# ZYM-PKU/UDiffText

Measured on AMD Instinct MI355X. Metric: 512x512 50-step denoised images/sec (UDiffText hot path: conditioner + 50 CFG Euler steps + VAE decode), higher is better.
Workload: dtype bf16; 1 GPU; 512x512, 50 Euler/DDIM(eta 0) steps, CFG 5.0, 9-char labels, noise_iters 0; global batch 4 per step sharded over 1 GPU(s) = 4 images per GPU in micro-batches of 4: every UNet call runs ONE batch of 4 (8 samples with CFG); 3 such batch(es) in flight per GPU on separate launch streams; BASELINE.json configs[1]; global_batch=4, weights=synthetic (name-keyed recipe), 1361.2 M parameters, launch=hipGraph replay of the sampler steps, in_flight=3, batches_per_unet_call=1

## Files before the change

udifftext_amd/csrc/gemm.hip:

```cpp
#include "common.h"
#include <stdio.h>
#include <stdlib.h>
#include <string.h>
#include <atomic>
#include <cmath>

hipError_t udt_lean_launch_gemm(int cfg, const void* lparams, int smem, int G, int geglu, int ln, hipStream_t s);
hipError_t udt_lean_launch_conv3(const void* c3params, hipStream_t s);

namespace {
#include "tile_common.h"

struct GemmParams {
  const uint16_t* a;
  const uint16_t* a2;
  const uint16_t* w;
  const uint16_t* zero;
  const float* bias;
  const uint16_t* res;
  const float* rowvec;
  void* out;
  const float* colscale;
  const float* in_scsh;
  float* colstats;
// ... 709 lines not shown
  if ((reinterpret_cast<uintptr_t>(d->a) | reinterpret_cast<uintptr_t>(d->w) | reinterpret_cast<uintptr_t>(d->out)) & 15) return false;
  return true;
}

bool lean_plan(const udt_gemm_desc* d, LeanPlan& t, bool want_stats) {
  const int mode = lean_mode();
  if (mode == 0) return false;
  constexpr int unsupported = UDT_GEMM_OUT_F32 | UDT_GEMM_RELU | UDT_GEMM_TRANSPOSED | UDT_GEMM_SILU_OUT;
  if (d->flags & unsupported) return false;
  const bool conv1 = (d->flags & UDT_GEMM_CONV) != 0;
  if (conv1 && (d->ksize != 1 || d->stride != 1 || d->upsample || d->pad_t != 0 || d->pad_l != 0 || d->Hout != d->Hin ||
                d->Wout != d->Win || d->C1 % BK != 0 || d->C2 % BK != 0 || d->ln_colsum || (d->flags & UDT_GEMM_GEGLU)))
    return false;
  const bool mx8 = (d->flags & UDT_GEMM_MX8) != 0;
  const bool emit = d->q8_out != nullptr;
  if (d->batch > 1 || d->in_scsh || (d->colscale != nullptr) != mx8) return false;
  const bool geglu = (d->flags & UDT_GEMM_GEGLU) != 0;
  const bool ln = d->ln_colsum != nullptr;
  if (want_stats && (geglu || ln || !lean_stats_enabled())) return false;
  if (mx8 || emit) {
    if (conv1 || d->rowvec || mode == 0 || (mode > 0 && mode != 1)) return false;
    if (mx8 && (!d->a_scale || d->K % 128 != 0 || d->lda % 16 != 0 || (d->ldw > 0 && d->ldw % 16 != 0))) return false;
    if (mx8 && ln && (!d->rowstat_in || d->rowstat_in_parts <= 0)) return false;
    if (!mx8 && geglu) return false;
    if (mx8 && geglu && !(ln && emit)) return false;
    if (mx8 && !geglu && ln && emit && d->rowstat_out) return false;
    if (emit && (want_stats || !d->q8_scale || d->ld_q8 % 8 != 0 || d->N % (geglu ? 64 : 32) != 0)) return false;
    if (d->rowstat_out && (!emit || geglu)) return false;
    if (d->q8_fixed_col > 0 && (!emit || geglu || d->q8_fixed_col % 32 != 0 || !(d->q8_fixed_mul > 0.f))) return false;
    if ((reinterpret_cast<uintptr_t>(d->q8_out) | reinterpret_cast<uintptr_t>(d->colscale)) & 15) return false;
  } else if (d->rowstat_out || d->rowstat_in) {
    return false;
  }
// ... 36 lines not shown
  if (!geglu && d->N % 160 == 0 && d->N % 128 != 0 && t.cfg == 1) t.cfg = 5;
  if (mode <= 0 && d->N >= 768 && (long long)((d->M + 255) / 256) * ((d->N + 255) / 256) >= 2LL * device_cus() &&
      (d->cu_share <= 1 || lean256_under_lanes())) t.cfg = 6;
  }
  t.stats_rows = 0;
  if (want_stats) {
    if (t.cfg != 1 && t.cfg != 5) {
      if (mode > 0) return false;
      t.cfg = (d->N % 160 == 0 && d->N % 128 != 0) ? 5 : 1;
    }
    if (mx8) t.cfg = 1;
    t.stats_rows = t.cfg == 1 ? 64 : 32;
    const int rpb = d->rows_per_batch > 0 ? d->rows_per_batch : d->M;
    if (rpb % t.stats_rows != 0) return false;
  }
  switch (t.cfg) {
    case 1: t.nw = 4; t.bm = 128; t.bn = 128; t.smem = 2 * (128 + 128) * ROW_BYTES; break;
    case 5: t.nw = 4; t.bm = 128; t.bn = 160; t.smem = 128 * 160 * 4; break;
    case 6: t.nw = 8; t.bm = 256; t.bn = 256; t.smem = 2 * (256 + 256) * ROW_BYTES; break;
    default: return false;
  }
  {
    const int epi = (t.cfg == 6 ? t.bm * t.bn : t.bm * t.bn * 4) + ((ln && t.cfg != 5) ? t.bm * 8 : 0);
    if (t.smem < epi) t.smem = epi;
  }
  t.tiles_m = (d->M + t.bm - 1) / t.bm;
  t.tiles_n = (d->N + t.bn - 1) / t.bn;
  t.tiles = t.tiles_m * t.tiles_n;
  t.nkt = d->K / KT;
  int slots = device_cus() * ((t.cfg == 1 || t.cfg == 5) ? 2 : 1) / share_of(d);
  if (slots < 1) slots = 1;
  int sk = 1;
// ... 210 lines not shown
  LeanPlan lt;
  return lean_plan(d, lt, d->colstats != nullptr) ? 1 : 0;
}

extern "C" int32_t udt_gemm_rowstat_parts(const udt_gemm_desc* d) {
  if (!d || d->M <= 0 || d->N <= 0 || d->K <= 0) return 0;
  udt_gemm_desc t = *d;
  alignas(16) static const uint64_t probe_dst[2] = {0, 0};
  if (!t.q8_out) { t.q8_out = const_cast<uint64_t*>(probe_dst); t.q8_scale = const_cast<uint64_t*>(probe_dst); if (t.ld_q8 <= 0) t.ld_q8 = (t.N + 15) / 16 * 16; }
  LeanPlan lt;
  if (!lean_plan(&t, lt, false) || lt.cfg != 1 || (d->flags & UDT_GEMM_GEGLU)) return 0;
  return (d->N + 63) / 64;
}
extern "C" int32_t udt_gemm_in_scsh_ok(const udt_gemm_desc* d) {
  if (!d || d->K <= 0 || d->K % BK != 0) return 0;
  c3p::Geo ge;
  return conv3p_geometry(d, ge, true) ? 1 : 0;
}

extern "C" int32_t udt_gemm_up4_ok(const udt_gemm_desc* d) {
  if (!d || d->upsample != 2) return 0;
  lg::C3Params c3;
  return lean_conv_plan(d, c3, d->colstats != nullptr) ? 1 : 0;
}

extern "C" int udt_gn_silu_conv3x3_fwd(const udt_gemm_desc* d, void* workspace, size_t workspace_bytes, void* stream) {
  if (!d || !(d->flags & UDT_GEMM_CONV) || d->ksize != 3 || d->stride != 1 || d->pad_t != 1 || d->pad_l != 1 || !d->in_scsh)
    return UDT_ERR_BAD_ARG;
  return udt_gemm(d, workspace, workspace_bytes, stream);
}
// ... 23 lines not shown
    }
  }
  if (use_gemm8(d)) {
    TilePlan t8 = plan_tiles8(d);
    if (!t8.fixup) return 0;
    return G8_HEADER_BYTES + (size_t)t8.G * t8.bm * t8.bn * sizeof(float);
  }
  TilePlan t = plan_tiles(d);
  if (t.bm != 256 || !t.fixup) return 0;
  return G8_HEADER_BYTES + (size_t)t.G * 2 * SLAB_FLOATS * sizeof(float);
}

extern "C" int udt_gemm(const udt_gemm_desc* d, void* workspace, size_t workspace_bytes, void* stream) {
  if (!d || !d->a || !d->w) return UDT_ERR_BAD_ARG;
  if (d->M <= 0 || d->N <= 0 || d->K <= 0) return UDT_ERR_BAD_SHAPE;
  if (d->K % k_tile(d) != 0) return UDT_ERR_BAD_SHAPE;
  if (d->N % 4 != 0) return UDT_ERR_BAD_SHAPE;
  const bool mx8 = (d->flags & UDT_GEMM_MX8) != 0;
  if (mx8 || d->q8_out || d->rowstat_out || d->rowstat_in) {
    LeanPlan lt8;
    if (!lean_plan(d, lt8, d->colstats != nullptr)) return UDT_ERR_BAD_ARG;
  } else if (d->colscale) {
    return UDT_ERR_BAD_ARG;
  }
  const bool conv = (d->flags & UDT_GEMM_CONV) != 0;
  const bool trans = (d->flags & UDT_GEMM_TRANSPOSED) != 0;
  const int batch = d->batch > 0 ? d->batch : 1;
  if (conv) {
    if (d->ksize != 1 && d->ksize != 3) return UDT_ERR_BAD_SHAPE;
    if (d->C1 <= 0 || d->C1 % BK != 0 || d->C2 % BK != 0) return UDT_ERR_BAD_SHAPE;
// ... 97 lines not shown
      lp.kt_split = (conv1 && d->C2 > 0) ? d->C1 / BK : lt.nkt;
      lp.a2_bytes = (unsigned)((long long)d->M * (conv1 ? d->C2 : 0) * 2);
      lp.alpha = d->alpha; lp.ln_eps = d->ln_eps;
      lp.tiles_m = lt.tiles_m; lp.tiles_n = lt.tiles_n; lp.n_block = lt.n_block; lp.tiles = lt.tiles;
      lp.nkt = lt.nkt; lp.splitk = lt.splitk; lp.kt_per = lt.kt_per;
      lp.a_bytes = (unsigned)((long long)d->M * lp.lda * elem_bytes(d));
      lp.w_bytes = (unsigned)((long long)d->N * p.ldw * elem_bytes(d));
      lp.a_scale = mx8 ? reinterpret_cast<const uint32_t*>(d->a_scale) : nullptr;
      lp.colscale = d->colscale;
      lp.rowstat_in = d->rowstat_in; lp.rowstat_in_parts = d->rowstat_in_parts;
      lp.q8_out = reinterpret_cast<uint8_t*>(d->q8_out); lp.q8_scale = reinterpret_cast<uint32_t*>(d->q8_scale); lp.ld_q8 = d->ld_q8;
      lp.rowstat_out = d->rowstat_out;
      lp.q8_fixed_col = d->q8_fixed_col > 0 ? d->q8_fixed_col : 0x7fffffff;
      lp.q8_fixed_mul = d->q8_fixed_mul;
      lp.G = lt.G;
      lp.counters = nullptr; lp.slabs = nullptr;
      if (lt.splitk > 1) {
        if (!workspace || workspace_bytes < lean_workspace(lt)) return UDT_ERR_WORKSPACE;
        lp.counters = reinterpret_cast<int*>(workspace);
        lp.slabs = reinterpret_cast<float*>(reinterpret_cast<char*>(workspace) + G8_HEADER_BYTES);
      }
      UdtProfScope profl(cls, s);
      if (profl.rec) {
        char tag[96];
        snprintf(tag, sizeof(tag), "lean%d%s%s M=%d N=%d K=%d fl=0x%x ln=%d tile=%dx%d units=%d splitk=%d", lt.cfg, mx8 ? "-mx8" : "", d->q8_out ? "+q8" : "",
                 d->M, d->N, d->K, d->flags, d->ln_colsum ? 1 : 0, lt.bm, lt.bn, lt.tiles * lt.splitk, lt.splitk);
        udt_prof_tag(profl.rec, tag);
      }
      const bool geglu = (d->flags & UDT_GEMM_GEGLU) != 0, ln = d->ln_colsum != nullptr;
      hipError_t el;
      el = udt_lean_launch_gemm(lt.cfg, &lp, lt.smem, lt.G, geglu ? 1 : 0, ln ? 1 : 0, s);
      if (el != hipSuccess) return udt_set_hip_error(el);
      return UDT_OK;
    }
  }
  if (d->ln_colsum) return UDT_ERR_BAD_ARG;
  {
    lg::C3Params c3;
    if (lean_conv_plan(d, c3, d->colstats != nullptr)) {
      c3.colstats = d->colstats;
      c3.a = p.a; c3.w = p.w; c3.bias = p.bias; c3.res = p.res; c3.rowvec = p.rowvec; c3.out = reinterpret_cast<uint16_t*>(d->out);
// ... 145 lines not shown
```

udifftext_amd/csrc/lean.h:

```cpp
#pragma once

namespace lg {

using g8::wait_vm;
UDT_DEVINL void raw_barrier() {
  asm volatile("s_waitcnt lgkmcnt(0)" ::: "memory");
  __builtin_amdgcn_s_barrier();
  asm volatile("" ::: "memory");
}
using g8::buf_lds16;
using g8::OOB;

typedef __attribute__((ext_vector_type(2))) __bf16 bf2_t;
UDT_DEVINL float dot2_bf16(uint32_t a, uint32_t b, float c) {
  return __builtin_amdgcn_fdot2_f32_bf16(__builtin_bit_cast(bf2_t, a), __builtin_bit_cast(bf2_t, b), c, false);
}

template <int CPR, int RPI>
UDT_DEVINL void wave_colstats(char* wl, int lane, const float (&cs)[8], const float (&cq)[8], float* dst, bool col_ok) {
#pragma unroll
  for (int h = 0; h < 2; ++h) {
    f32x4 a = {cs[4 * h + 0], cs[4 * h + 1], cs[4 * h + 2], cs[4 * h + 3]};
    f32x4 b = {cq[4 * h + 0], cq[4 * h + 1], cq[4 * h + 2], cq[4 * h + 3]};
    *reinterpret_cast<f32x4*>(wl + lane * 64 + h * 16) = a;
// ... 12 lines not shown
        const f32x4 a = *reinterpret_cast<const f32x4*>(src + h * 16);
        const f32x4 b = *reinterpret_cast<const f32x4*>(src + 32 + h * 16);
#pragma unroll
        for (int e = 0; e < 4; ++e) { ts[4 * h + e] += a[e]; tq[4 * h + e] += b[e]; }
      }
    }
#pragma unroll
    for (int h = 0; h < 4; ++h) {
      f32x4 v = {ts[2 * h], tq[2 * h], ts[2 * h + 1], tq[2 * h + 1]};
      *reinterpret_cast<f32x4*>(dst + h * 4) = v;
    }
  }
}

template <int NW, int WGM, int WGN, int TM, int TN, int NST, bool GEGLU, bool LN, int TMB = TM, bool STATS = false, bool FP8 = false,
          bool EMIT = false>
__global__ void __launch_bounds__(NW * 64, 2) lgemm_kernel(const LParams p) {
  static_assert(!STATS || (!GEGLU && !LN), "statistics-emitting epilogue: plain linears / 1x1 convolutions");
  static_assert(!FP8 || NST == 2, "the fp8 loop is written for the two-stage ring");
  static_assert(!EMIT || (TN * 4) % 4 == 0, "a 32-column block = 4 lanes of the row layout");
  constexpr int EB = FP8 ? 1 : 2;
  static_assert(TM % TMB == 0, "epilogue passes of TMB row tiles");
  static_assert(WGM * WGN == NW, "wave grid");
  static_assert(!GEGLU || TN == 2, "GEGLU pairs the two 32-column tiles of a wave");
  constexpr int BM = WGM * TM * 32, BN = WGN * TN * 32;
  constexpr int A_BYTES = BM * ROW_BYTES, B_BYTES = BN * ROW_BYTES, STAGE_BYTES = A_BYTES + B_BYTES;
  constexpr int A_PIECES = BM / 8, B_PIECES = BN / 8;
  constexpr int A_INSTR = (A_PIECES + NW - 1) / NW, B_INSTR = (B_PIECES + NW - 1) / NW;
  constexpr int LPT = A_INSTR + B_INSTR;
  constexpr int WROWS = TM * 32, WCOLS = TN * 32;
  constexpr int EROW = WCOLS * 4;
  constexpr int EPI_WAVE = TMB * 32 * EROW;
// ... 47 lines not shown
    const int koff = (pslot ^ ((row >> 1) & 7)) * 8;
    const int m = m0 + row;
    a_voff[i] = (m < p.M) ? (unsigned)((long long)m * p.lda * EB + koff * 2) : OOB;
    a2_voff[i] = (m < p.M) ? (unsigned)(((long long)m * p.lda2 + koff) * 2) : OOB;
  }
#pragma unroll
  for (int i = 0; i < B_INSTR; ++i) {
    int idx = wave + NW * i;
    while (idx >= B_PIECES) idx -= NW;
    w_piece[i] = idx;
    const int row = idx * 8 + l3;
    const int koff = (pslot ^ ((row >> 1) & 7)) * 8;
    const int n = n0 + row;
    w_voff[i] = (n < p.N) ? (unsigned)((long long)n * p.ldw * EB + koff * 2) : OOB;
  }
  auto stage = [&](int st, int kt) {
    char* abuf = smem + st * STAGE_BYTES;
    char* bbuf = abuf + A_BYTES;
    if (kt < p.kt_split) {
#pragma unroll
      for (int i = 0; i < A_INSTR; ++i) buf_lds16(rsrc_a, abuf + a_piece[i] * 1024, a_voff[i], kt * ROW_BYTES);
    } else {
#pragma unroll
      for (int i = 0; i < A_INSTR; ++i) buf_lds16(rsrc_a2, abuf + a_piece[i] * 1024, a2_voff[i], (kt - p.kt_split) * ROW_BYTES);
    }
#pragma unroll
    for (int i = 0; i < B_INSTR; ++i) buf_lds16(rsrc_w, bbuf + w_piece[i] * 1024, w_voff[i], kt * ROW_BYTES);
  };

#pragma unroll
  for (int s = 0; s < NST - 1; ++s)
    if (s < nk) stage(s, kreal(s));
  const uint32_t* asp[TM];
  uint32_t asc_nxt[TM];
  if constexpr (FP8) {
#pragma unroll
    for (int tm = 0; tm < TM; ++tm) {
      int m = m0 + row0 + tm * 32 + l31;
      if (m >= p.M) m = p.M - 1;
      asp[tm] = p.a_scale + m;
      asc_nxt[tm] = (nk > 0) ? asp[tm][(long long)kreal(0) * p.M] : 0x7f7f7f7fu;
    }
// ... 71 lines not shown
        for (int tn = 0; tn < TN; ++tn) acc[tm][tn] = mfma32_mx8<2>(wf[1][tn], xf[1][tm], acc[tm][tn], asc[tm]);
      if constexpr (TM * TN <= 5) {
        __builtin_amdgcn_sched_group_barrier(0x100, 4 * (TM + TN), 0);
        __builtin_amdgcn_sched_group_barrier(0x008, 2 * TM * TN, 0);
      }
    } else {
    bf16x8_t xf[4][TM], wf[4][TN];
#pragma unroll
    for (int ks = 0; ks < 4; ++ks) {
      const int slot = ((ks * 2 + hi) ^ swz) << 4;
#pragma unroll
      for (int t = 0; t < TM; ++t) xf[ks][t] = lds_read_frag(abuf + a_frag_row + t * 32 * ROW_BYTES + slot);
#pragma unroll
      for (int t = 0; t < TN; ++t) wf[ks][t] = lds_read_frag(bbuf + b_frag_row + t * 32 * ROW_BYTES + slot);
    }
#pragma unroll
    for (int ks = 0; ks < 4; ++ks) {
#pragma unroll
      for (int tm = 0; tm < TM; ++tm)
#pragma unroll
        for (int tn = 0; tn < TN; ++tn) acc[tm][tn] = mfma32(wf[ks][tn], xf[ks][tm], acc[tm][tn]);
      if constexpr (LN) {
        if (wn == 0) {
#pragma unroll
          for (int tm = 0; tm < TM; ++tm) {
            const u32x4 v = __builtin_bit_cast(u32x4, xf[ks][tm]);
#pragma unroll
            for (int j = 0; j < 4; ++j) {
              rs[tm] = dot2_bf16(v[j], 0x3f803f80u, rs[tm]);
              rq[tm] = dot2_bf16(v[j], v[j], rq[tm]);
            }
          }
        }
      }
    }
    if constexpr (TM * TN <= 5) {
      __builtin_amdgcn_sched_group_barrier(0x100, 4 * (TM + TN), 0);
      __builtin_amdgcn_sched_group_barrier(0x008, 4 * TM * TN, 0);
    }
    }
    st = st + 1;
    if (st >= NST) st = 0;
  }
  raw_barrier();

  if (p.splitk > 1) {
    f32x4* slab = reinterpret_cast<f32x4*>(p.slabs + (long long)unit * (BM * BN));
#pragma unroll
    for (int tm = 0; tm < TM; ++tm)
#pragma unroll
      for (int tn = 0; tn < TN; ++tn)
// ... 668 lines not shown
```

udifftext_amd/csrc/lean.hip:

```cpp
#include "common.h"
#include <stdio.h>
#include <stdlib.h>
#include <atomic>

namespace {
#include "tile_common.h"
#include "lean_params.h"
#include "lean.h"
#include "wide.h"
#include "rowres.h"

template <int NW, int WGM, int WGN, int TM, int TN, int NST, int TMB = TM>
hipError_t launch_lean(const lg::LParams& lp, int smem, int G, bool geglu, bool ln, hipStream_t s) {
  static AttrOnce once[5];
  const void* fn;
  const bool stats = lp.colstats != nullptr;
  if constexpr (NW == 4 && NST == 2) {
    if (stats) {
      fn = (const void*)lg::lgemm_kernel<NW, WGM, WGN, TM, TN, NST, false, false, TMB, true>;
      hipError_t e = once[4].ensure(fn, smem);
      if (e != hipSuccess) return e;
      void* args[] = {const_cast<lg::LParams*>(&lp)};
      return hipLaunchKernel(fn, dim3(G), dim3(NW * 64), args, smem, s);
    }
  }
  if (stats) return hipErrorInvalidValue;
  if constexpr (TN == 2) {
    fn = geglu ? (ln ? (const void*)lg::lgemm_kernel<NW, WGM, WGN, TM, TN, NST, true, true, TMB> : (const void*)lg::lgemm_kernel<NW, WGM, WGN, TM, TN, NST, true, false, TMB>)
               : (ln ? (const void*)lg::lgemm_kernel<NW, WGM, WGN, TM, TN, NST, false, true, TMB> : (const void*)lg::lgemm_kernel<NW, WGM, WGN, TM, TN, NST, false, false, TMB>);
  } else {
    fn = ln ? (const void*)lg::lgemm_kernel<NW, WGM, WGN, TM, TN, NST, false, true, TMB> : (const void*)lg::lgemm_kernel<NW, WGM, WGN, TM, TN, NST, false, false, TMB>;
  }
  hipError_t e = once[(geglu ? 2 : 0) + (ln ? 1 : 0)].ensure(fn, smem);
  if (e != hipSuccess) return e;
  void* args[] = {const_cast<lg::LParams*>(&lp)};
  return hipLaunchKernel(fn, dim3(G), dim3(NW * 64), args, smem, s);
}

template <bool GEGLU, bool LN, bool STATS, bool FP8, bool EMIT>
hipError_t launch_lean_mx8_k(const lg::LParams& lp, int smem, int G, hipStream_t s) {
  static AttrOnce once;
// ... 83 lines not shown
```

udifftext_amd/csrc/lean_params.h:

```cpp
#pragma once

namespace lg {

struct LParams {
  const uint16_t* a;
  const uint16_t* a2;
  const uint16_t* w;
  const float* bias;
  const uint16_t* res;
  const float* rowvec;
  const float* ln_s;
  uint16_t* out;
  int M, N, K;
  int lda, ldw, ldo, ldr, ldrv, rows_per_batch;
  float alpha, ln_eps;
  int tiles_m, tiles_n, n_block, tiles;
  int nkt;
  int splitk, kt_per;
  unsigned a_bytes, w_bytes;
  int kt_split, lda2;
  unsigned a2_bytes;
  int G;
  int* counters;
  float* slabs;
  float* colstats;
  const uint32_t* a_scale;
  const float* colscale;
  const float* rowstat_in;
  int rowstat_in_parts;
  uint8_t* q8_out;
  uint32_t* q8_scale;
  int ld_q8;
  int q8_fixed_col;
  float q8_fixed_mul;
  float* rowstat_out;
};

struct C3Params {
  const uint16_t* a;
  const uint16_t* w;
  const float* bias;
  const uint16_t* res;
  const float* rowvec;
  uint16_t* out;
  int N, C;
  int B, H, W;
  int ldw, ldo, ldr, ldrv;
  float alpha;
  int tiles_x, tiles_y, tiles_m, tiles_n, n_block, tiles;
  int chunks, splitk, ch_per;
// ... 13 lines not shown
```

udifftext_amd/ops.py:

```python
from __future__ import annotations

import contextlib
import ctypes as C
import os
import threading
from typing import NamedTuple, Optional, Sequence

import torch

from . import lib as L

WORKSPACE_BYTES = 96 << 20


class Workspace:

    def __init__(self, device, nbytes: int = WORKSPACE_BYTES):
        if torch.device(device).type != "cuda":
            raise L.UdtError("udifftext_amd workspaces live on the GPU (no CPU fallback)")
        self.buf = torch.zeros(nbytes, dtype=torch.uint8, device=device)

    def check(self, stream: Optional[int] = None) -> None:
        L.check(L.load().udt_check_async_error(self.buf.data_ptr(), self.buf.numel(), _stream() if stream is None else stream),
                "udt_check_async_error")
# ... 59 lines not shown


def _bf16(t: torch.Tensor) -> None:
    if t.dtype != torch.bfloat16:
        raise ValueError(f"expected bf16 tensor, got {t.dtype}")


def gemm_desc(**kw) -> L.GemmDesc:
    d = L.GemmDesc()
    d.batch = 1
    d.alpha = 1.0
    d.cu_share = _ctx.cu_share
    for k, v in kw.items():
        setattr(d, k, v)
    return d


def run_gemm(d: L.GemmDesc, device, fused_gn: bool = False) -> None:
    lib = L.load()
    need = lib.udt_gemm_workspace_bytes(C.byref(d))
    ws_ptr, ws_bytes = None, 0
    if need:
        ws = _ws(need, device)
        ws_ptr, ws_bytes = ws.data_ptr(), ws.numel()
    if fused_gn:
        L.check(lib.udt_gn_silu_conv3x3_fwd(C.byref(d), ws_ptr, ws_bytes, _stream()), "udt_gn_silu_conv3x3_fwd")
    else:
        L.check(lib.udt_gemm(C.byref(d), ws_ptr, ws_bytes, _stream()), "udt_gemm")


# ... 49 lines not shown
    lib = L.load()
    parts = lib.udt_gemm_rowstat_parts(C.byref(d)) if rowstats else 0
    if not lib.udt_gemm_q8_ok(C.byref(d)) or (rowstats and parts <= 0):
        d.q8_out, d.q8_scale, d.ld_q8, d.q8_fixed_col = None, None, 0, 0
        return None
    if rowstats:
        st = torch.empty((parts, M, 2), dtype=torch.float32, device=device)
        d.rowstat_out = st.data_ptr()
        q = Mx8Act(q.data, q.scale, st)
    return q


def linear(x: torch.Tensor, w: torch.Tensor, bias: Optional[torch.Tensor] = None, *, out: Optional[torch.Tensor] = None,
           residual: Optional[torch.Tensor] = None, rowvec: Optional[torch.Tensor] = None, rows_per_batch: int = 0,
           flags: int = 0, alpha: float = 1.0, n_out: Optional[int] = None, colstats: bool = False,
           emit_q8: bool = False, emit_rowstats: bool = False) -> torch.Tensor:
    _bf16(x); _bf16(w)
    K = x.shape[-1]
    x2 = x.reshape(-1, K) if x.is_contiguous() else x
    assert x2.dim() == 2 and x2.stride(1) == 1
    M = x2.shape[0]
    N = w.shape[0] if n_out is None else n_out
    assert w.shape[1] == K and w.is_contiguous()
    n_cols = N // 2 if (flags & L.GEMM_GEGLU) else N
    if out is None:
        dt = torch.float32 if (flags & L.GEMM_OUT_F32) else torch.bfloat16
        if flags & L.GEMM_TRANSPOSED:
            assert rows_per_batch > 0
            out = torch.empty((M // rows_per_batch, N, rows_per_batch), dtype=dt, device=x.device)
        else:
            out = torch.empty((M, n_cols), dtype=dt, device=x.device)
    ldo = out.stride(0) if not (flags & L.GEMM_TRANSPOSED) else 0
    d = gemm_desc(a=_ptr(x2), w=_ptr(w), bias=_ptr(bias), residual=_ptr(residual), rowvec=_ptr(rowvec), out=_ptr(out),
                  M=M, N=N, K=K, lda=x2.stride(0), ldo=ldo, ldr=(residual.stride(0) if residual is not None else 0),
                  rows_per_batch=rows_per_batch, ld_rowvec=(rowvec.stride(0) if rowvec is not None else 0), flags=flags,
                  alpha=alpha)
    if not (colstats and rows_per_batch > 0 and out.is_contiguous() and _attach_colstats(d, out, n_cols, rows_per_batch)):
        _drop_stale_stats(out)
    q8 = None
    if emit_q8 and not (flags & (L.GEMM_OUT_F32 | L.GEMM_TRANSPOSED | L.GEMM_GEGLU)) and d.colstats is None and rowvec is None:
        q8 = _attach_q8(d, M, n_cols, x.device, emit_rowstats)
    run_gemm(d, x.device)
    if getattr(out, "mx8", None) is not None:
        del out.mx8
    if q8 is not None:
        out.mx8 = q8
    if WORK_COUNTER is not None:
        count_work("gemm", 2.0 * M * N * K)
        count_work("gemm_bytes", 2.0 * (M * K + N * K) + out.numel() * out.element_size()
                   + (2.0 * M * n_cols if residual is not None else 0.0))
        count_work("gemm_launches", 1.0)
# ... 128 lines not shown
        assert x2.is_contiguous() and x2.shape[:3] == x.shape[:3]
        C2 = x2.shape[3]
    Hv, Wv = (H * 2, W_ * 2) if upsample else (H, W_)
    if pad is None:
        pad = (ksize // 2, ksize // 2)
    if out_hw is None:
        out_hw = ((Hv + 2 * pad[0] - ksize) // stride + 1, (Wv + 2 * pad[1] - ksize) // stride + 1)
    Ho, Wo = out_hw
    N = w.shape[0] if n_out is None else n_out
    K = ksize * ksize * (C1 + C2)
    assert w.shape[1] == K, (w.shape, K)
    M = B * Ho * Wo
    if out is None and not probe_in_scsh:
        dt = torch.float32 if (flags & L.GEMM_OUT_F32) else torch.bfloat16
        out = torch.empty((B, Ho, Wo, N), dtype=dt, device=x.device)
    d = gemm_desc(a=_ptr(x), a2=_ptr(x2), w=_ptr(w), bias=_ptr(bias), residual=_ptr(residual), rowvec=_ptr(rowvec),
                  out=_ptr(out), M=M, N=N, K=K, lda=0, ldo=(out.stride(2) if out is not None else N),
                  ldr=(residual.stride(2) if residual is not None else 0),
                  Hin=H, Win=W_, C1=C1, C2=C2, Hout=Ho, Wout=Wo, ksize=ksize, stride=stride, pad_t=pad[0], pad_l=pad[1],
                  upsample=1 if upsample else 0, rows_per_batch=Ho * Wo,
                  ld_rowvec=(rowvec.stride(0) if rowvec is not None else 0), flags=flags | L.GEMM_CONV)
    if probe_in_scsh:
        return bool(L.load().udt_gemm_in_scsh_ok(C.byref(d)))
    if w_up4 is not None and upsample and ksize == 3 and x2 is None and in_scsh is None:
        _bf16(w_up4)
        assert w_up4.is_contiguous() and w_up4.dim() == 3 and w_up4.shape[0] == 4 and w_up4.shape[1] >= N and w_up4.shape[2] == 4 * C1, \
            (w_up4.shape, N, C1)
        d.upsample, d.w, d.ldw, d.stride_w = 2, _ptr(w_up4), w_up4.shape[2], w_up4.stride(0)
        if not L.load().udt_gemm_up4_ok(C.byref(d)):
            d.upsample, d.w, d.ldw, d.stride_w = 1, _ptr(w), 0, 0
    if in_scsh is not None:
        assert in_scsh.dtype == torch.float32 and in_scsh.is_contiguous() and in_scsh.numel() == B * (C1 + C2) * 2
        d.in_scsh = in_scsh.data_ptr()
        d.in_act = int(in_act)
    if not (colstats and _attach_colstats(d, out, N, Ho * Wo)):
        _drop_stale_stats(out)
    if in_scsh is not None:
        run_gemm(d, x.device, fused_gn=True)
    else:
        run_gemm(d, x.device)
    return out


def attention(q: torch.Tensor, k: torch.Tensor, vt: torch.Tensor, heads: int, scale: float,
              out: Optional[torch.Tensor] = None) -> torch.Tensor:
    _bf16(q); _bf16(k); _bf16(vt)
    B, Nq = q.shape[0], q.shape[1]
    Nk = k.shape[1]
    assert q.stride(2) == 1 and k.stride(2) == 1 and vt.stride(2) == 1
    if out is None:
        out = torch.empty((B, Nq, heads * 64), dtype=torch.bfloat16, device=q.device)
    L.check(L.load().udt_attn_fwd(_ptr(q), _ptr(k), _ptr(vt), _ptr(out), B, heads, Nq, Nk,
                                  q.stride(1), k.stride(1), vt.stride(1), out.stride(1),
# ... 814 lines not shown
```

udifftext_amd/sgm/modules/attention.py:

```python
from __future__ import annotations

import os
from typing import List, Optional

import torch
import torch.nn as nn

from udifftext_amd import ops, packing

from . import hipnn as H
from .diffusionmodules.util import zero_module


TATTN_FUSED = True

FF_PROJ = os.environ.get("UDT_FF_PROJ", "1") != "0"


class GEGLU(H._Packed):
    def __init__(self, dim_in: int, dim_out: int):
        super().__init__()
        self.proj = H.Linear(dim_in, dim_out * 2)

    def _sources(self):
# ... 249 lines not shown
        self.proj_out = zero_module(H.Linear(inner, in_channels))
        self.use_linear = use_linear

    def project_context(self, context_bf16) -> List[torch.Tensor]:
        return [blk.t_attn.project_context(context_bf16) for blk in self.transformer_blocks]

    def prepare_fused(self, kv_list, out=None) -> list:
        return [blk.t_attn.prepare_fused(kv, blk.t_norm, out=(out[i] if out is not None else None))
                for i, (blk, kv) in enumerate(zip(self.transformer_blocks, kv_list))]

    def forward(self, x, t_context=None, v_context=None, t_kv: Optional[list] = None, emit_map: bool = False,
                zero_ctx_rows: int = 0, t_fused: Optional[list] = None):
        B, Hh, Ww, C = x.shape
        N = Hh * Ww
        mx = H.mx8_width(self.proj_in.out_features)
        t2 = self.proj_in(self.norm(x).reshape(B * N, C), emit_q8=mx, emit_rowstats=mx)
        t = H.carry_mx8(t2.reshape(B, N, -1), t2)
        nb = len(self.transformer_blocks)
        defer = FF_PROJ and H.LN_GEMM and not mx
        for i, blk in enumerate(self.transformer_blocks):
            t = blk(t, t_context=t_context, t_kv=(t_kv[i] if t_kv is not None else None), emit_map=emit_map,
                    zero_ctx_rows=zero_ctx_rows, t_fused=(t_fused[i] if t_fused is not None else None),
                    x8=ops.mx8_of(t) if mx else None, emit_rowstats=(i + 1 < nb), defer_ff_out=(defer and i + 1 == nb),
                    hw=(Hh, Ww))
        if isinstance(t, tuple):
            hid, t3 = t
            w, b = self.packed_ffproj()
            st = H.want_stats(B, N, w.shape[0])
            out = ops.conv2d(hid.reshape(B, Hh, Ww, -1), w, b, x2=t3.reshape(B, Hh, Ww, -1), ksize=1, pad=(0, 0), residual=x,
                             n_out=w.shape[0], colstats=st)
            if ops.WORK_COUNTER is not None:
# ... 29 lines not shown
```

udifftext_amd/sgm/modules/hipnn.py:

```python
from __future__ import annotations

import math
import os
from typing import Optional

import torch
import torch.nn as nn

from udifftext_amd import lib as L
from udifftext_amd import ops, packing

from ..util import init_skipped


def count_flops(kind: str, flops: float) -> None:
    ops.count_work(kind, flops)


FUSE_GN = os.environ.get("UDT_FUSE_GN", "0") != "0"

GN_EPI = os.environ.get("UDT_GN_EPI", "1") != "0" and os.environ.get("UDT_LEAN", "") != "0"
EMIT_STATS = FUSE_GN or GN_EPI


def want_stats(B: int, HW: int, C: int) -> bool:
    return FUSE_GN or (GN_EPI and C % 8 == 0)


FP8_LINEARS = os.environ.get("UDT_FP8", "0") != "0"


FP8_ATTENTION = os.environ.get("UDT_FP8_ATTN", "1") != "0"


def fp8_attention() -> bool:
    return FP8_LINEARS and LN_GEMM and FP8_ATTENTION

# ... 106 lines not shown
        _init_uniform_(self.weight, in_features)
        if bias:
            self.bias = nn.Parameter(torch.empty(out_features))
            _init_uniform_(self.bias, in_features)
        else:
            self.register_parameter("bias", None)

    def _pack(self):
        return packing.pack_linear(self.weight), packing.pad_bias(self.bias)

    def _pack_fp8(self):
        wq, cs = packing.pack_linear_fp8(self.weight)
        return wq, cs, packing.pad_bias(self.bias)

    def forward(self, x, residual=None, flags: int = 0, out=None, rowvec=None, rows_per_batch: int = 0,
                colstats: bool = False, x8=None, emit_q8: bool = False, emit_rowstats: bool = False):
        if x8 is not None:
            wq, cs, b = self.packed_fp8()
            M = x8.data.shape[0]
            if colstats:
                rpb = rows_per_batch if rows_per_batch > 0 else M
                colstats = want_stats(M // rpb, rpb, wq.shape[0])
            return ops.linear_mx8(x8, wq, cs, b, residual=residual, flags=flags, out=out, rows_per_batch=rows_per_batch,
                                  colstats=bool(colstats), emit_q8=emit_q8, emit_rowstats=emit_rowstats)
        w, b = self.packed()
        if colstats:
            rpb = rows_per_batch if rows_per_batch > 0 else x.shape[0]
            colstats = want_stats(x.shape[0] // rpb, rpb, w.shape[0])
        return ops.linear(x, w, b, residual=residual, flags=flags, out=out, rowvec=rowvec, rows_per_batch=rows_per_batch,
                          colstats=bool(colstats), emit_q8=emit_q8, emit_rowstats=emit_rowstats)


class Conv2d(_Packed):

    def __init__(self, in_channels: int, out_channels: int, kernel_size: int, stride: int = 1, padding: int = 0):
        super().__init__()
        self.in_channels, self.out_channels = in_channels, out_channels
        self.kernel_size, self.stride, self.padding = kernel_size, stride, padding
        self.weight = nn.Parameter(torch.empty(out_channels, in_channels, kernel_size, kernel_size))
        self.bias = nn.Parameter(torch.empty(out_channels))
        fan_in = in_channels * kernel_size * kernel_size
        _init_uniform_(self.weight, fan_in)
        _init_uniform_(self.bias, fan_in)
        self.segments = None
        self.n_pad = 4
# ... 65 lines not shown
        self.weight = nn.Parameter(torch.ones(num_channels))
        self.bias = nn.Parameter(torch.zeros(num_channels))

    def forward(self, x, x2=None, silu: bool = False):
        if GN_EPI:
            st1, st2 = ops.gn_stats_of(x), ops.gn_stats_of(x2)
            C1, C2 = x.shape[-1], (x2.shape[-1] if x2 is not None else 0)
            HW = x.numel() // (x.shape[0] * C1)
            if (st1 is not None and (x2 is None or st2 is not None)
                    and (ops.gn_strip_ok(x.shape[0], HW, C1, C2, self.num_groups)
                         or ((C1 + C2) % 64 == 0 and (C1 + C2) // self.num_groups <= 128))):
                count_flops("gn_from_epilogue_stats", 1)
                return ops.group_norm_from_stats(x, st1, self.weight, self.bias, self.num_groups, self.eps, silu, x2=x2, st2=st2)
        return ops.group_norm(x, self.weight, self.bias, self.num_groups, self.eps, silu, x2=x2)


class LayerNorm(nn.Module):
    def __init__(self, dim: int, eps: float = 1e-5):
        super().__init__()
        self.dim, self.eps = dim, eps
        self.weight = nn.Parameter(torch.ones(dim))
        self.bias = nn.Parameter(torch.zeros(dim))

    def forward(self, x):
        return ops.layer_norm(x, self.weight, self.bias, self.eps)


def fuse_rows(*weights: torch.Tensor) -> torch.Tensor:
    return packing.pack_linear(torch.cat(list(weights), dim=0))

# ... 7 lines not shown
```

Before: 10.62 images/s.

## Fuse GroupNorm affine into proj_in GEMM A-fragment loads

Adds a GNA variant of the lean bf16 GEMM kernel that stages per-batch GroupNorm scale/shift tables into LDS and applies them to the A fragments before the MFMA. The spatial transformer's proj_in then runs as a 1x1 conv that takes the finalized GN table from epilogue stats, skipping the separate GroupNorm kernel and its full activation write and read. The cost is extra LDS traffic, per-fragment FMA work, and dropping the scheduling barrier hints in the inner loop. Tiles are also restricted to the 128-row configs.

Measured after the change: 10.67 images/s (median of 6 runs). No clear change (+0.5%).

```diff
diff --git a/udifftext_amd/csrc/gemm.hip b/udifftext_amd/csrc/gemm.hip
--- a/udifftext_amd/csrc/gemm.hip
+++ b/udifftext_amd/csrc/gemm.hip
@@ -747,9 +747,14 @@
     return false;
   const bool mx8 = (d->flags & UDT_GEMM_MX8) != 0;
   const bool emit = d->q8_out != nullptr;
-  if (d->batch > 1 || d->in_scsh || (d->colscale != nullptr) != mx8) return false;
+  if (d->batch > 1 || (d->colscale != nullptr) != mx8) return false;
   const bool geglu = (d->flags & UDT_GEMM_GEGLU) != 0;
   const bool ln = d->ln_colsum != nullptr;
+  const bool gna = d->in_scsh != nullptr;
+  if (gna && ((conv1 && d->C2 != 0) || mx8 || emit || geglu || ln || want_stats || d->in_act != 0 || d->rows_per_batch < 64 ||
+              d->M % d->rows_per_batch != 0 || (reinterpret_cast<uintptr_t>(d->in_scsh) & 15) ||
+              (long long)(d->M / d->rows_per_batch) * (d->K / BK) * 512 >= (1LL << 31)))
+    return false;
   if (want_stats && (geglu || ln || !lean_stats_enabled())) return false;
   if (mx8 || emit) {
     if (conv1 || d->rowvec || mode == 0 || (mode > 0 && mode != 1)) return false;
@@ -816,8 +821,9 @@
     const int rpb = d->rows_per_batch > 0 ? d->rows_per_batch : d->M;
     if (rpb % t.stats_rows != 0) return false;
   }
+  if (gna && t.cfg != 1 && t.cfg != 5) return false;
   switch (t.cfg) {
-    case 1: t.nw = 4; t.bm = 128; t.bn = 128; t.smem = 2 * (128 + 128) * ROW_BYTES; break;
+    case 1: t.nw = 4; t.bm = 128; t.bn = 128; t.smem = 2 * (128 + 128) * ROW_BYTES + (gna ? 2 * lg::GNA_STAGE_BYTES : 0); break;
     case 5: t.nw = 4; t.bm = 128; t.bn = 160; t.smem = 128 * 160 * 4; break;
     case 6: t.nw = 8; t.bm = 256; t.bn = 256; t.smem = 2 * (256 + 256) * ROW_BYTES; break;
     default: return false;
@@ -1058,6 +1064,14 @@
 }
 extern "C" int32_t udt_gemm_in_scsh_ok(const udt_gemm_desc* d) {
   if (!d || d->K <= 0 || d->K % BK != 0) return 0;
+  if (d->M > 0 && d->N > 0) {
+    udt_gemm_desc t = *d;
+    alignas(16) static const float probe_table[4] = {0.f, 0.f, 0.f, 0.f};
+    if (!t.in_scsh) t.in_scsh = probe_table;
+    LeanPlan lt;
+    if (lean_plan(&t, lt, t.colstats != nullptr)) return 1;
+  }
+  if (!(d->flags & UDT_GEMM_CONV)) return 0;
   c3p::Geo ge;
   return conv3p_geometry(d, ge, true) ? 1 : 0;
 }
@@ -1111,6 +1125,7 @@
 extern "C" int udt_gemm(const udt_gemm_desc* d, void* workspace, size_t workspace_bytes, void* stream) {
   if (!d || !d->a || !d->w) return UDT_ERR_BAD_ARG;
   if (d->M <= 0 || d->N <= 0 || d->K <= 0) return UDT_ERR_BAD_SHAPE;
+  if (d->in_scsh && !(d->flags & UDT_GEMM_CONV) && !udt_gemm_in_scsh_ok(d)) return UDT_ERR_BAD_ARG;
   if (d->K % k_tile(d) != 0) return UDT_ERR_BAD_SHAPE;
   if (d->N % 4 != 0) return UDT_ERR_BAD_SHAPE;
   const bool mx8 = (d->flags & UDT_GEMM_MX8) != 0;
@@ -1238,6 +1253,8 @@
       lp.q8_fixed_col = d->q8_fixed_col > 0 ? d->q8_fixed_col : 0x7fffffff;
       lp.q8_fixed_mul = d->q8_fixed_mul;
       lp.G = lt.G;
+      lp.in_scsh = d->in_scsh;
+      lp.scsh_bytes = d->in_scsh ? (unsigned)((long long)(d->M / p.rows_per_batch) * lt.nkt * 512) : 0u;
       lp.counters = nullptr; lp.slabs = nullptr;
       if (lt.splitk > 1) {
         if (!workspace || workspace_bytes < lean_workspace(lt)) return UDT_ERR_WORKSPACE;
@@ -1247,8 +1264,8 @@
       UdtProfScope profl(cls, s);
       if (profl.rec) {
         char tag[96];
-        snprintf(tag, sizeof(tag), "lean%d%s%s M=%d N=%d K=%d fl=0x%x ln=%d tile=%dx%d units=%d splitk=%d", lt.cfg, mx8 ? "-mx8" : "", d->q8_out ? "+q8" : "",
-                 d->M, d->N, d->K, d->flags, d->ln_colsum ? 1 : 0, lt.bm, lt.bn, lt.tiles * lt.splitk, lt.splitk);
+        snprintf(tag, sizeof(tag), "lean%d%s%s M=%d N=%d K=%d fl=0x%x ln=%d tile=%dx%d units=%d splitk=%d%s", lt.cfg, mx8 ? "-mx8" : "", d->q8_out ? "+q8" : "",
+                 d->M, d->N, d->K, d->flags, d->ln_colsum ? 1 : 0, lt.bm, lt.bn, lt.tiles * lt.splitk, lt.splitk, d->in_scsh ? " gn" : "");
         udt_prof_tag(profl.rec, tag);
       }
       const bool geglu = (d->flags & UDT_GEMM_GEGLU) != 0, ln = d->ln_colsum != nullptr;
diff --git a/udifftext_amd/csrc/lean.h b/udifftext_amd/csrc/lean.h
--- a/udifftext_amd/csrc/lean.h
+++ b/udifftext_amd/csrc/lean.h
@@ -50,8 +50,10 @@
 }
 
 template <int NW, int WGM, int WGN, int TM, int TN, int NST, bool GEGLU, bool LN, int TMB = TM, bool STATS = false, bool FP8 = false,
-          bool EMIT = false>
+          bool EMIT = false, bool GNA = false>
 __global__ void __launch_bounds__(NW * 64, 2) lgemm_kernel(const LParams p) {
+  static_assert(!GNA || (!GEGLU && !LN && !STATS && !FP8 && !EMIT && NW == 4 && NST == 2 && WGM * TM * 32 == 128),
+                "GroupNorm on the A fragments: the plain bf16 128-row two-stage kernels");
   static_assert(!STATS || (!GEGLU && !LN), "statistics-emitting epilogue: plain linears / 1x1 convolutions");
   static_assert(!FP8 || NST == 2, "the fp8 loop is written for the two-stage ring");
   static_assert(!EMIT || (TN * 4) % 4 == 0, "a 32-column block = 4 lanes of the row layout");
@@ -129,6 +131,24 @@
     const int n = n0 + row;
     w_voff[i] = (n < p.N) ? (unsigned)((long long)n * p.ldw * EB + koff * 2) : OOB;
   }
+  const __amdgpu_buffer_rsrc_t rsrc_gn =
+      __builtin_amdgcn_make_buffer_rsrc(const_cast<float*>(GNA ? p.in_scsh : nullptr), 0, GNA ? p.scsh_bytes : 0u, 0x00020000);
+  unsigned gn_voff = OOB;
+  int gn_off[TM];
+#pragma unroll
+  for (int tm = 0; tm < TM; ++tm) gn_off[tm] = 0;
+  if constexpr (GNA) {
+    const int gn_b0 = m0 / p.rows_per_batch;
+    const int nb = p.M / p.rows_per_batch;
+    const int bs = gn_b0 + 2 * wave + hi;
+    if (wave < GNA_NS / 2 && bs < nb) gn_voff = (unsigned)(((long long)bs * p.nkt) * 512 + l31 * 16);
+#pragma unroll
+    for (int tm = 0; tm < TM; ++tm) {
+      int m = m0 + row0 + tm * 32 + l31;
+      if (m >= p.M) m = p.M - 1;
+      gn_off[tm] = (m / p.rows_per_batch - gn_b0) * 512;
+    }
+  }
   auto stage = [&](int st, int kt) {
     char* abuf = smem + st * STAGE_BYTES;
     char* bbuf = abuf + A_BYTES;
@@ -141,6 +161,9 @@
     }
 #pragma unroll
     for (int i = 0; i < B_INSTR; ++i) buf_lds16(rsrc_w, bbuf + w_piece[i] * 1024, w_voff[i], kt * ROW_BYTES);
+    if constexpr (GNA) {
+      if (wave < GNA_NS / 2) buf_lds16(rsrc_gn, smem + NST * STAGE_BYTES + st * GNA_STAGE_BYTES + wave * 1024, gn_voff, kt * 512);
+    }
   };
 
 #pragma unroll
@@ -242,6 +265,23 @@
 #pragma unroll
       for (int t = 0; t < TN; ++t) wf[ks][t] = lds_read_frag(bbuf + b_frag_row + t * 32 * ROW_BYTES + slot);
     }
+    if constexpr (GNA) {
+      const char* tab = smem + NST * STAGE_BYTES + st * GNA_STAGE_BYTES;
+#pragma unroll
+      for (int ks = 0; ks < 4; ++ks)
+#pragma unroll
+        for (int tm = 0; tm < TM; ++tm) {
+          const char* tp = tab + gn_off[tm] + (ks * 2 + hi) * 32;
+          const f32x4 sc0 = *reinterpret_cast<const f32x4*>(tp), sc1 = *reinterpret_cast<const f32x4*>(tp + 16);
+          const f32x4 sh0 = *reinterpret_cast<const f32x4*>(tp + 256), sh1 = *reinterpret_cast<const f32x4*>(tp + 272);
+          u32x4 v = __builtin_bit_cast(u32x4, xf[ks][tm]);
+          v[0] = pack_bf16x2(bf16_lo(v[0]) * sc0[0] + sh0[0], bf16_hi(v[0]) * sc0[1] + sh0[1]);
+          v[1] = pack_bf16x2(bf16_lo(v[1]) * sc0[2] + sh0[2], bf16_hi(v[1]) * sc0[3] + sh0[3]);
+          v[2] = pack_bf16x2(bf16_lo(v[2]) * sc1[0] + sh1[0], bf16_hi(v[2]) * sc1[1] + sh1[1]);
+          v[3] = pack_bf16x2(bf16_lo(v[3]) * sc1[2] + sh1[2], bf16_hi(v[3]) * sc1[3] + sh1[3]);
+          xf[ks][tm] = __builtin_bit_cast(bf16x8_t, v);
+        }
+    }
 #pragma unroll
     for (int ks = 0; ks < 4; ++ks) {
 #pragma unroll
@@ -262,7 +302,7 @@
         }
       }
     }
-    if constexpr (TM * TN <= 5) {
+    if constexpr (TM * TN <= 5 && !GNA) {
       __builtin_amdgcn_sched_group_barrier(0x100, 4 * (TM + TN), 0);
       __builtin_amdgcn_sched_group_barrier(0x008, 4 * TM * TN, 0);
     }
diff --git a/udifftext_amd/csrc/lean.hip b/udifftext_amd/csrc/lean.hip
--- a/udifftext_amd/csrc/lean.hip
+++ b/udifftext_amd/csrc/lean.hip
@@ -12,10 +12,18 @@
 
 template <int NW, int WGM, int WGN, int TM, int TN, int NST, int TMB = TM>
 hipError_t launch_lean(const lg::LParams& lp, int smem, int G, bool geglu, bool ln, hipStream_t s) {
-  static AttrOnce once[5];
+  static AttrOnce once[6];
   const void* fn;
   const bool stats = lp.colstats != nullptr;
   if constexpr (NW == 4 && NST == 2) {
+    if (lp.in_scsh) {
+      if (stats || geglu || ln) return hipErrorInvalidValue;
+      fn = (const void*)lg::lgemm_kernel<NW, WGM * TM, 1, 1, WGN * TN, NST, false, false, 1, false, false, false, true>;
+      hipError_t e = once[5].ensure(fn, smem);
+      if (e != hipSuccess) return e;
+      void* args[] = {const_cast<lg::LParams*>(&lp)};
+      return hipLaunchKernel(fn, dim3(G), dim3(NW * 64), args, smem, s);
+    }
     if (stats) {
       fn = (const void*)lg::lgemm_kernel<NW, WGM, WGN, TM, TN, NST, false, false, TMB, true>;
       hipError_t e = once[4].ensure(fn, smem);
@@ -24,7 +32,7 @@
       return hipLaunchKernel(fn, dim3(G), dim3(NW * 64), args, smem, s);
     }
   }
-  if (stats) return hipErrorInvalidValue;
+  if (stats || lp.in_scsh) return hipErrorInvalidValue;
   if constexpr (TN == 2) {
     fn = geglu ? (ln ? (const void*)lg::lgemm_kernel<NW, WGM, WGN, TM, TN, NST, true, true, TMB> : (const void*)lg::lgemm_kernel<NW, WGM, WGN, TM, TN, NST, true, false, TMB>)
                : (ln ? (const void*)lg::lgemm_kernel<NW, WGM, WGN, TM, TN, NST, false, true, TMB> : (const void*)lg::lgemm_kernel<NW, WGM, WGN, TM, TN, NST, false, false, TMB>);
diff --git a/udifftext_amd/csrc/lean_params.h b/udifftext_amd/csrc/lean_params.h
--- a/udifftext_amd/csrc/lean_params.h
+++ b/udifftext_amd/csrc/lean_params.h
@@ -1,6 +1,9 @@
 #pragma once
 
 namespace lg {
+
+constexpr int GNA_NS = 4;
+constexpr int GNA_STAGE_BYTES = GNA_NS * 512;
 
 struct LParams {
   const uint16_t* a;
@@ -34,6 +37,8 @@
   int q8_fixed_col;
   float q8_fixed_mul;
   float* rowstat_out;
+  const float* in_scsh;
+  unsigned scsh_bytes;
 };
 
 struct C3Params {
diff --git a/udifftext_amd/ops.py b/udifftext_amd/ops.py
--- a/udifftext_amd/ops.py
+++ b/udifftext_amd/ops.py
@@ -97,6 +97,9 @@
     for k, v in kw.items():
         setattr(d, k, v)
     return d
+
+
+_probe_desc = gemm_desc
 
 
 def run_gemm(d: L.GemmDesc, device, fused_gn: bool = False) -> None:
@@ -176,7 +179,8 @@
 def linear(x: torch.Tensor, w: torch.Tensor, bias: Optional[torch.Tensor] = None, *, out: Optional[torch.Tensor] = None,
            residual: Optional[torch.Tensor] = None, rowvec: Optional[torch.Tensor] = None, rows_per_batch: int = 0,
            flags: int = 0, alpha: float = 1.0, n_out: Optional[int] = None, colstats: bool = False,
-           emit_q8: bool = False, emit_rowstats: bool = False) -> torch.Tensor:
+           emit_q8: bool = False, emit_rowstats: bool = False, in_scsh: Optional[torch.Tensor] = None,
+           probe_in_scsh: bool = False) -> torch.Tensor:
     _bf16(x); _bf16(w)
     K = x.shape[-1]
     x2 = x.reshape(-1, K) if x.is_contiguous() else x
@@ -185,6 +189,14 @@
     N = w.shape[0] if n_out is None else n_out
     assert w.shape[1] == K and w.is_contiguous()
     n_cols = N // 2 if (flags & L.GEMM_GEGLU) else N
+    if probe_in_scsh:
+        if colstats or emit_q8 or rows_per_batch <= 0:
+            return False
+        d = _probe_desc(a=_ptr(x2), w=_ptr(w), bias=_ptr(bias), residual=_ptr(residual), rowvec=_ptr(rowvec), M=M, N=N, K=K,
+                      lda=x2.stride(0), ldo=(out.stride(0) if out is not None else n_cols),
+                      ldr=(residual.stride(0) if residual is not None else 0), rows_per_batch=rows_per_batch,
+                      ld_rowvec=(rowvec.stride(0) if rowvec is not None else 0), flags=flags, alpha=alpha)
+        return bool(L.load().udt_gemm_in_scsh_ok(C.byref(d)))
     if out is None:
         dt = torch.float32 if (flags & L.GEMM_OUT_F32) else torch.bfloat16
         if flags & L.GEMM_TRANSPOSED:
@@ -197,6 +209,10 @@
                   M=M, N=N, K=K, lda=x2.stride(0), ldo=ldo, ldr=(residual.stride(0) if residual is not None else 0),
                   rows_per_batch=rows_per_batch, ld_rowvec=(rowvec.stride(0) if rowvec is not None else 0), flags=flags,
                   alpha=alpha)
+    if in_scsh is not None:
+        assert rows_per_batch > 0 and M % rows_per_batch == 0 and K % 64 == 0
+        assert in_scsh.dtype == torch.float32 and in_scsh.is_contiguous() and in_scsh.numel() == (M // rows_per_batch) * K * 2
+        d.in_scsh = in_scsh.data_ptr()
     if not (colstats and rows_per_batch > 0 and out.is_contiguous() and _attach_colstats(d, out, n_cols, rows_per_batch)):
         _drop_stale_stats(out)
     q8 = None
@@ -355,7 +371,8 @@
     if out is None and not probe_in_scsh:
         dt = torch.float32 if (flags & L.GEMM_OUT_F32) else torch.bfloat16
         out = torch.empty((B, Ho, Wo, N), dtype=dt, device=x.device)
-    d = gemm_desc(a=_ptr(x), a2=_ptr(x2), w=_ptr(w), bias=_ptr(bias), residual=_ptr(residual), rowvec=_ptr(rowvec),
+    d = (_probe_desc if probe_in_scsh else gemm_desc)(
+                  a=_ptr(x), a2=_ptr(x2), w=_ptr(w), bias=_ptr(bias), residual=_ptr(residual), rowvec=_ptr(rowvec),
                   out=_ptr(out), M=M, N=N, K=K, lda=0, ldo=(out.stride(2) if out is not None else N),
                   ldr=(residual.stride(2) if residual is not None else 0),
                   Hin=H, Win=W_, C1=C1, C2=C2, Hout=Ho, Wout=Wo, ksize=ksize, stride=stride, pad_t=pad[0], pad_l=pad[1],
@@ -377,7 +394,7 @@
     if not (colstats and _attach_colstats(d, out, N, Ho * Wo)):
         _drop_stale_stats(out)
     if in_scsh is not None:
-        run_gemm(d, x.device, fused_gn=True)
+        run_gemm(d, x.device, fused_gn=(ksize == 3))
     else:
         run_gemm(d, x.device)
     return out
diff --git a/udifftext_amd/sgm/modules/attention.py b/udifftext_amd/sgm/modules/attention.py
--- a/udifftext_amd/sgm/modules/attention.py
+++ b/udifftext_amd/sgm/modules/attention.py
@@ -287,7 +287,17 @@
         B, Hh, Ww, C = x.shape
         N = Hh * Ww
         mx = H.mx8_width(self.proj_in.out_features)
-        t2 = self.proj_in(self.norm(x).reshape(B * N, C), emit_q8=mx, emit_rowstats=mx)
+        pw, pb = self.proj_in.packed()
+        pkw = dict(ksize=1, pad=(0, 0), n_out=pw.shape[0])
+        if (H.GN_PROJ_IN and not mx and N >= H.GN_PROJ_IN_MIN_ROWS and self.norm.table_ok(x) and pw.shape[1] == C
+                and ops.conv2d(x, pw, pb, probe_in_scsh=True, **pkw)):
+            t2 = ops.conv2d(x, pw, pb, in_scsh=self.norm.table(x), in_act=0, **pkw).reshape(B * N, -1)
+            if ops.WORK_COUNTER is not None:
+                H.count_flops("gemm", 2.0 * B * N * pw.shape[0] * C)
+                H.count_flops("gemm_bytes", 2.0 * (B * N * C + pw.shape[0] * C) + 2.0 * B * N * pw.shape[0])
+                H.count_flops("gemm_launches", 1.0)
+        else:
+            t2 = self.proj_in(self.norm(x).reshape(B * N, C), emit_q8=mx, emit_rowstats=mx)
         t = H.carry_mx8(t2.reshape(B, N, -1), t2)
         nb = len(self.transformer_blocks)
         defer = FF_PROJ and H.LN_GEMM and not mx
diff --git a/udifftext_amd/sgm/modules/hipnn.py b/udifftext_amd/sgm/modules/hipnn.py
--- a/udifftext_amd/sgm/modules/hipnn.py
+++ b/udifftext_amd/sgm/modules/hipnn.py
@@ -21,6 +21,9 @@
 
 GN_EPI = os.environ.get("UDT_GN_EPI", "1") != "0" and os.environ.get("UDT_LEAN", "") != "0"
 EMIT_STATS = FUSE_GN or GN_EPI
+
+GN_PROJ_IN = os.environ.get("UDT_GN_PROJ_IN", "1") != "0"
+GN_PROJ_IN_MIN_ROWS = 128
 
 
 def want_stats(B: int, HW: int, C: int) -> bool:
@@ -157,7 +160,8 @@
         return wq, cs, packing.pad_bias(self.bias)
 
     def forward(self, x, residual=None, flags: int = 0, out=None, rowvec=None, rows_per_batch: int = 0,
-                colstats: bool = False, x8=None, emit_q8: bool = False, emit_rowstats: bool = False):
+                colstats: bool = False, x8=None, emit_q8: bool = False, emit_rowstats: bool = False, in_scsh=None,
+                probe_in_scsh: bool = False):
         if x8 is not None:
             wq, cs, b = self.packed_fp8()
             M = x8.data.shape[0]
@@ -171,7 +175,8 @@
             rpb = rows_per_batch if rows_per_batch > 0 else x.shape[0]
             colstats = want_stats(x.shape[0] // rpb, rpb, w.shape[0])
         return ops.linear(x, w, b, residual=residual, flags=flags, out=out, rowvec=rowvec, rows_per_batch=rows_per_batch,
-                          colstats=bool(colstats), emit_q8=emit_q8, emit_rowstats=emit_rowstats)
+                          colstats=bool(colstats), emit_q8=emit_q8, emit_rowstats=emit_rowstats, in_scsh=in_scsh,
+                          probe_in_scsh=probe_in_scsh)
 
 
 class Conv2d(_Packed):
@@ -267,6 +272,16 @@
                 return ops.group_norm_from_stats(x, st1, self.weight, self.bias, self.num_groups, self.eps, silu, x2=x2, st2=st2)
         return ops.group_norm(x, self.weight, self.bias, self.num_groups, self.eps, silu, x2=x2)
 
+    def table_ok(self, x) -> bool:
+        C = x.shape[-1]
+        return bool(GN_EPI and ops.gn_stats_of(x) is not None and C % 64 == 0 and C % self.num_groups == 0
+                    and C // self.num_groups <= 128)
+
+    def table(self, x) -> torch.Tensor:
+        B, C = x.shape[0], x.shape[-1]
+        return ops.gn_finalize(ops.gn_stats_of(x), C, None, 0, self.weight, self.bias, B, x.numel() // (B * C), self.num_groups,
+                               self.eps)
+
 
 class LayerNorm(nn.Module):
     def __init__(self, dim: int, eps: float = 1e-5):
```
